# CagriCatik/RRT-MPC

Measured on NVIDIA B200. Metric: MPC QP solves/sec (horizon 50, batched), higher is better.
Workload: dtype f64

## Files before the change

rrt_mpc_b200/csrc/mpc_core.h:

```cpp
#pragma once
#include <math.h>
#include <stdint.h>

#ifdef __CUDACC__
#define MPC_HD __host__ __device__ __forceinline__
#else
#define MPC_HD inline
#endif

namespace mpc {

struct Params {
  double L, dt;
  double pq[4][4], pr[2][2], pqn[4][4];
  double u_lo[2], u_hi[2];
  double v_lo, v_hi;
  double du_lo[2], du_hi[2];
  double w_v, w_u, w_du;
  int N;
};

struct Settings {
  double eps_abs, eps_rel;
  double rho0, alpha, sigma;
// ... 1106 lines not shown
    w.act()[N + 1] = ib;
  }
  return changed;
}

MPC_HD int activity_probe_stage(const View& w, const Params& p, int k) {
  const int N = w.N;
  const double* rc = w.rec(k);
  const int old = w.act()[k];
  int bits = 0;
  const int ng = ngroups(N, k);
  const double tol = 1e-6;
  for (int g = 0; g < ng; ++g) {
    double lo, hi; group_bounds(p, w.hdr(), k, g, lo, hi);
    const double m0 = rc[R_V + 3 * g] - hi, m1 = lo - rc[R_V + 3 * g + 1], m2 = -rc[R_V + 3 * g + 2];
    const int b0 = fabs(m0) <= tol ? (old >> (3 * g)) & 1 : (m0 > 0.0);
    const int b1 = fabs(m1) <= tol ? (old >> (3 * g + 1)) & 1 : (m1 > 0.0);
    const int b2 = fabs(m2) <= tol ? (old >> (3 * g + 2)) & 1 : (m2 > 0.0);
    bits |= (b0 << (3 * g)) | (b1 << (3 * g + 1)) | (b2 << (3 * g + 2));
  }
  if (k < N) bits |= 0xF << 15;
  int changed = (old != bits);
  w.act()[k] = bits;
  if (k == 0) {
    changed |= (w.act()[N + 1] != 0xF);
    w.act()[N + 1] = 0xF;
  }
  return changed;
}

struct PolishRP {
  View w; const Params* p; double inv_delta; int zero_sol;
  MPC_HD double dyn(int k, int r) const {
    if (!act_dyn_bit(w, k, r)) return 0.0;
    const double* rc = w.rec(k);
    double b = r == 0 ? rc[R_LIN + 5] : (r == 1 ? rc[R_LIN + 6] : 0.0);
    double z[4]; StateXV xs{w}; dyn_rows(w, *p, k, xs, z);
    return (b - z[r]) * inv_delta - rc[R_YE + r];
  }
  MPC_HD double init(int r) const {
    if (!act_init_bit(w, r)) return 0.0;
    const double* h = w.hdr();
    return (h[H_X0 + r] - w.rec(0)[R_XU + r]) * inv_delta - h[H_YI + r];
  }
  MPC_HD double row(int k, int g, int r) const {
    if (!((act_group_bits(w, k, g) >> r) & 1)) return 0.0;
    double lo, hi; group_bounds(*p, w.hdr(), k, g, lo, hi);
    StateXV xs{w};
    const double* rc = w.rec(k);
    double gv = group_g(k, g, xs), sv = rc[R_S + g];
    double ax = r == 0 ? gv - sv : (r == 1 ? gv + sv : sv);
    double b = r == 0 ? hi : (r == 1 ? lo : 0.0);
    return (b - ax) * inv_delta - rc[R_V + 3 * g + r];
  }
  MPC_HD void group_vals(int k, int g, const Mode& m, double& rr_s, double& gval) const {
    double v1 = row(k, g, 0), v2 = row(k, g, 1), v3 = row(k, g, 2);
    double ps = group_ps(*p, g);
    GroupCoef c = group_coef(m, ps, act_group_bits(w, k, g));
    rr_s = -ps * w.rec(k)[R_S + g] + (-v1 + v2 + v3);
    gval = v1 + v2 - c.csg * c.mss_inv * rr_s;
  }
  Mode mode;
  MPC_HD double grp(int k, int g) const { double a, b; group_vals(k, g, mode, a, b); return b; }
};

MPC_HD void polish_rhs_stage(const View& w, const Params& p, const Mode& m, int k) {
  const int N = w.N;
  double* rc = w.rec(k);
  PolishRP rp{w, &p, m.inv_delta, 0, m};
  const int ng = ngroups(N, k);
  for (int g = 0; g < ng; ++g) {
    double rr_s, gval; rp.group_vals(k, g, m, rr_s, gval);
    rc[R_ST + g] = rr_s;
  }
  double out[6];
  gather_xu(w, p, k, rp, out);
  const int nj = k < N ? 6 : 4;
  for (int j = 0; j < nj; ++j) {
    double qj = j < 4 ? rc[R_Q + j] : 0.0;
    w.bx_set(k, j, -qj - px_entry(p, k < N, j, rc + R_XU) + out[j]);
  }
  for (int j = nj; j < 6; ++j) w.bx_set(k, j, 0.0);
}
MPC_HD void polish_dual_stage(const View& w, const Params& p, const Mode& m, int k) {
  const int N = w.N;
  double* rc = w.rec(k);
  BxXV dx{w};
  StateXV xs{w};
  const int ng = ngroups(N, k);
  for (int g = 0; g < ng; ++g) {
    double lo, hi; group_bounds(p, w.hdr(), k, g, lo, hi);
    int bits = act_group_bits(w, k, g);
    GroupCoef c = group_coef(m, group_ps(p, g), bits);
    double gd = group_g(k, g, dx);
    double ds = (rc[R_ST + g] - c.csg * gd) * c.mss_inv;
    rc[R_ST + g] = ds;
    double gv = group_g(k, g, xs), sv = rc[R_S + g];
    double ax[3] = {gv - sv, gv + sv, sv};
    double ad[3] = {gd - ds, gd + ds, ds};
    double b[3] = {hi, lo, 0.0};
    for (int r = 0; r < 3; ++r)
      if ((bits >> r) & 1) rc[R_V + 3 * g + r] += m.inv_delta * (ad[r] - (b[r] - ax[r]));
  }
  if (k < N) {
    double ax[4], ad[4]; dyn_rows(w, p, k, xs, ax); dyn_rows(w, p, k, dx, ad);
    double b[4] = {rc[R_LIN + 5], rc[R_LIN + 6], 0.0, 0.0};
    for (int r = 0; r < 4; ++r)
      if (act_dyn_bit(w, k, r)) rc[R_YE + r] += m.inv_delta * (ad[r] - (b[r] - ax[r]));
  }
  if (k == 0) {
    double* h = w.hdr();
    for (int r = 0; r < 4; ++r)
      if (act_init_bit(w, r)) h[H_YI + r] += m.inv_delta * (dx(0, r) - (h[H_X0 + r] - xs(0, r)));
  }
}
MPC_HD void polish_primal_stage(const View& w, int k) {
  double* rc = w.rec(k);
  const int nj = k < w.N ? 6 : 4;
  for (int j = 0; j < nj; ++j) rc[R_XU + j] += w.bx_get(k, j);
  const int ng = ngroups(w.N, k);
  for (int g = 0; g < ng; ++g) rc[R_S + g] += rc[R_ST + g];
}
MPC_HD void polish_zero_stage(const View& w, int k) {
  double* rc = w.rec(k);
  for (int j = 0; j < 11; ++j) rc[R_XU + j] = 0.0;
  for (int j = 0; j < 15; ++j) rc[R_V + j] = 0.0;
  for (int r = 0; r < 4; ++r) rc[R_YE + r] = 0.0;
  if (k == 0) for (int r = 0; r < 4; ++r) w.hdr()[H_YI + r] = 0.0;
}

struct PolConst {
  double invd;
  double lo[5], hi[5], ps[5];
  double mssinv[5][4];
  double up0, up1;
};
MPC_HD PolConst pol_const(const View& w, const Params& p, const Settings& s) {
  PolConst c;
  c.invd = 1.0 / s.delta;
  c.lo[0] = p.v_lo; c.hi[0] = p.v_hi;
  c.lo[1] = p.u_lo[0]; c.hi[1] = p.u_hi[0]; c.lo[2] = p.u_lo[1]; c.hi[2] = p.u_hi[1];
  c.lo[3] = p.du_lo[0]; c.hi[3] = p.du_hi[0]; c.lo[4] = p.du_lo[1]; c.hi[4] = p.du_hi[1];
  for (int g = 0; g < 5; ++g) {
    c.ps[g] = group_ps(p, g);
    for (int na = 0; na < 4; ++na) c.mssinv[g][na] = s.delta / ((c.ps[g] + s.delta) * s.delta + na);
  }
  c.up0 = w.hdr()[H_UPREV]; c.up1 = w.hdr()[H_UPREV + 1];
  return c;
}
MPC_HD double mss_pick(const PolConst& c, int g, int bits) {
  const int na = (bits & 1) + ((bits >> 1) & 1) + ((bits >> 2) & 1);
  return na == 0 ? c.mssinv[g][0] : (na == 1 ? c.mssinv[g][1] : (na == 2 ? c.mssinv[g][2] : c.mssinv[g][3]));
}
MPC_HD double pol_group_val(const PolConst& c, int g, int bits, double gv, double sv, double lo, double hi,
                            double y0, double y1, double y2, double& rr_s) {
  const double v0 = (bits & 1) ? fma(hi - (gv - sv), c.invd, -y0) : 0.0;
  const double v1 = (bits & 2) ? fma(lo - (gv + sv), c.invd, -y1) : 0.0;
  const double v2 = (bits & 4) ? fma(-sv, c.invd, -y2) : 0.0;
  rr_s = fma(-c.ps[g], sv, (v1 - v0) + v2);
  const double csg = (double)(((bits >> 1) & 1) - (bits & 1)) * c.invd;
  return (v0 + v1) - csg * mss_pick(c, g, bits) * rr_s;
}
MPC_HD void dyn_rows6(const double* lin, double dt, const double* x, const double* xn, double* z) {
  z[0] = xn[0] - (x[0] + lin[0] * x[2] + lin[1] * x[3]);
  z[1] = xn[1] - (x[1] + lin[2] * x[2] + lin[3] * x[3]);
  z[2] = xn[2] - (x[2] + lin[4] * x[5]);
  z[3] = xn[3] - (x[3] + dt * x[4]);
}

MPC_HD void polish_rhs_fast(const View& w, const Params& p, const PolConst& c, int k) {
  const int N = w.N;
  double* rc = w.rec(k);
  const bool reg = k < N;
  const int act = w.act()[k];
  double x[6];
#pragma unroll
  for (int j = 0; j < 6; ++j) x[j] = rc[R_XU + j];
  double out[6] = {0.0, 0.0, 0.0, 0.0, 0.0, 0.0};
  double ua = 0.0, ud = 0.0;
  if (k >= 1) {
    const double* rp = w.rec(k - 1);
    double xp[6], z[4];
#pragma unroll
    for (int j = 0; j < 6; ++j) xp[j] = rp[R_XU + j];
    ua = xp[4]; ud = xp[5];
    dyn_rows6(rp + R_LIN, p.dt, xp, x, z);
    const int ap = w.act()[k - 1];
    const double b[4] = {rp[R_LIN + 5], rp[R_LIN + 6], 0.0, 0.0};
#pragma unroll
    for (int r = 0; r < 4; ++r) out[r] = ((ap >> (15 + r)) & 1) ? fma(b[r] - z[r], c.invd, -rp[R_YE + r]) : 0.0;
  } else {
    const double* h = w.hdr();
    const int ai = w.act()[N + 1];
#pragma unroll
    for (int r = 0; r < 4; ++r) out[r] = ((ai >> r) & 1) ? fma(h[H_X0 + r] - x[r], c.invd, -h[H_YI + r]) : 0.0;
  }
  const double off0 = k == 0 ? c.up0 : 0.0, off1 = k == 0 ? c.up1 : 0.0;
  const double gv[5] = {x[3], x[4], x[5], x[4] - (reg ? ua : 0.0), x[5] - (reg ? ud : 0.0)};
  const double offs[5] = {0.0, 0.0, 0.0, off0, off1};
  double G[5] = {0.0, 0.0, 0.0, 0.0, 0.0};
#pragma unroll
  for (int g = 0; g < 5; ++g) {
    if (g == 0 || reg) {
      double rr_s;
      G[g] = pol_group_val(c, g, (act >> (3 * g)) & 7, gv[g], rc[R_S + g], c.lo[g] + offs[g], c.hi[g] + offs[g],
                           rc[R_V + 3 * g], rc[R_V + 3 * g + 1], rc[R_V + 3 * g + 2], rr_s);
      rc[R_ST + g] = rr_s;
    }
  }
  out[3] += G[0];
  if (reg) {
    const double* rn = w.rec(k + 1);
    double xn[6], z[4];
#pragma unroll
    for (int j = 0; j < 6; ++j) xn[j] = rn[R_XU + j];
    const double* lin = rc + R_LIN;
    dyn_rows6(lin, p.dt, x, xn, z);
    const double b[4] = {lin[5], lin[6], 0.0, 0.0};
    double d[4];
#pragma unroll
    for (int r = 0; r < 4; ++r) d[r] = ((act >> (15 + r)) & 1) ? fma(b[r] - z[r], c.invd, -rc[R_YE + r]) : 0.0;
    out[0] -= d[0];
    out[1] -= d[1];
    out[2] -= lin[0] * d[0] + lin[2] * d[1] + d[2];
    out[3] -= lin[1] * d[0] + lin[3] * d[1] + d[3];
    out[4] = G[1] + G[3] - p.dt * d[3];
    out[5] = G[2] + G[4] - lin[4] * d[2];
    if (k + 1 < N) {
      const int an = w.act()[k + 1];
#pragma unroll
      for (int i = 0; i < 2; ++i) {
        double rr_s;
        out[4 + i] -= pol_group_val(c, 3 + i, (an >> (3 * (3 + i))) & 7, xn[4 + i] - x[4 + i], rn[R_S + 3 + i], c.lo[3 + i], c.hi[3 + i],
                                    rn[R_V + 3 * (3 + i)], rn[R_V + 3 * (3 + i) + 1], rn[R_V + 3 * (3 + i) + 2], rr_s);
      }
    }
  }
  int rev; double* bp = bx_ptr(w, k, rev);
#pragma unroll
  for (int j = 0; j < 6; ++j) {
    double val = 0.0;
    if (j < 4 || reg) val = -(j < 4 ? rc[R_Q + j] : 0.0) - px_entry(p, reg, j, x) + out[j];
    bp[rev ? 5 - j : j] = val;
  }
  if (k == mid_stage(N)) {
    double* bb = w.bottom().bx(N - k);
#pragma unroll
    for (int j = 0; j < 6; ++j) bb[j] = 0.0;
  }
}

MPC_HD void polish_dual_fast(const View& w, const Params& p, const PolConst& c, int k) {
  const int N = w.N;
  double* rc = w.rec(k);
  const bool reg = k < N;
  const int act = w.act()[k];
  double x[6], dx[6];
#pragma unroll
  for (int j = 0; j < 6; ++j) x[j] = rc[R_XU + j];
  bx_load6(w, k, dx);
  double ua = 0.0, ud = 0.0, dua_ = 0.0, dud_ = 0.0;
  if (k >= 1 && reg) {
    const double* rp = w.rec(k - 1);
    ua = rp[R_XU + 4]; ud = rp[R_XU + 5];
    double dp[6]; bx_load6(w, k - 1, dp); dua_ = dp[4]; dud_ = dp[5];
  }
  const double off0 = k == 0 ? c.up0 : 0.0, off1 = k == 0 ? c.up1 : 0.0;
  const double offs[5] = {0.0, 0.0, 0.0, off0, off1};
  const double gv[5] = {x[3], x[4], x[5], x[4] - ua, x[5] - ud};
  const double gd[5] = {dx[3], dx[4], dx[5], dx[4] - dua_, dx[5] - dud_};
#pragma unroll
  for (int g = 0; g < 5; ++g) {
    if (g == 0 || reg) {
      const int bits = (act >> (3 * g)) & 7;
      const double csg = (double)(((bits >> 1) & 1) - (bits & 1)) * c.invd;
      const double ds = (rc[R_ST + g] - csg * gd[g]) * mss_pick(c, g, bits);
      rc[R_ST + g] = ds;
      const double sv = rc[R_S + g];
      if (bits & 1) rc[R_V + 3 * g] += c.invd * ((gd[g] - ds) - ((c.hi[g] + offs[g]) - (gv[g] - sv)));
      if (bits & 2) rc[R_V + 3 * g + 1] += c.invd * ((gd[g] + ds) - ((c.lo[g] + offs[g]) - (gv[g] + sv)));
      if (bits & 4) rc[R_V + 3 * g + 2] += c.invd * (ds - (0.0 - sv));
    }
  }
  if (reg) {
    const double* rn = w.rec(k + 1);
    double xn[6], dn[6], ax[4], ad[4];
#pragma unroll
    for (int j = 0; j < 6; ++j) xn[j] = rn[R_XU + j];
    bx_load6(w, k + 1, dn);
    const double* lin = rc + R_LIN;
    dyn_rows6(lin, p.dt, x, xn, ax);
    dyn_rows6(lin, p.dt, dx, dn, ad);
    const double b[4] = {lin[5], lin[6], 0.0, 0.0};
#pragma unroll
    for (int r = 0; r < 4; ++r)
      if ((act >> (15 + r)) & 1) rc[R_YE + r] += c.invd * (ad[r] - (b[r] - ax[r]));
  }
  if (k == 0) {
    double* h = w.hdr();
    const int ai = w.act()[N + 1];
#pragma unroll
    for (int r = 0; r < 4; ++r)
      if ((ai >> r) & 1) h[H_YI + r] += c.invd * (dx[r] - (h[H_X0 + r] - x[r]));
  }
}

MPC_HD void residual_fast(const View& w, const Params& p, const IterConst& c, int ymode, int k, double* r) {
  const int N = w.N;
  const double* rc = w.rec(k);
  const bool reg = k < N;
  double x[6];
#pragma unroll
  for (int j = 0; j < 6; ++j) x[j] = rc[R_XU + j];
  double aty[6] = {0.0, 0.0, 0.0, 0.0, 0.0, 0.0};
  double ua = 0.0, ud = 0.0;
  if (k >= 1) {
    const double* rp = w.rec(k - 1);
    ua = rp[R_XU + 4]; ud = rp[R_XU + 5];
#pragma unroll
    for (int q = 0; q < 4; ++q) aty[q] = rp[R_YE + q];
  } else {
    const double* h = w.hdr();
#pragma unroll
    for (int q = 0; q < 4; ++q) {
      aty[q] = h[H_YI + q];
      const double ax = x[q], b = h[H_X0 + q];
      r[0] = dmax(r[0], fabs(ax - b)); r[1] = dmax(r[1], fabs(ax)); r[2] = dmax(r[2], fabs(b));
    }
  }
  const double off0 = k == 0 ? c.up0 : 0.0, off1 = k == 0 ? c.up1 : 0.0;
  const double offs[5] = {0.0, 0.0, 0.0, off0, off1};
  const double gv[5] = {x[3], x[4], x[5], x[4] - (reg ? ua : 0.0), x[5] - (reg ? ud : 0.0)};
  double Gy[5] = {0.0, 0.0, 0.0, 0.0, 0.0};
#pragma unroll
  for (int g = 0; g < 5; ++g) {
    if (g == 0 || reg) {
      const double hi = c.hi[g] + offs[g], lo = c.lo[g] + offs[g];
      const double sv = rc[R_S + g];
      const double v0 = rc[R_V + 3 * g], v1 = rc[R_V + 3 * g + 1], v2 = rc[R_V + 3 * g + 2];
      const double ax0 = gv[g] - sv, ax1 = gv[g] + sv, ax2 = sv;
      double z0, z1, z2, y0, y1, y2;
      if (ymode) { z0 = dmin2(ax0, hi); z1 = dmax2(ax1, lo); z2 = dmax2(ax2, 0.0); y0 = v0; y1 = v1; y2 = v2; }
      else {
        z0 = dmin2(v0, hi); z1 = dmax2(v1, lo); z2 = dmax2(v2, 0.0);
        y0 = c.rho * (v0 - z0); y1 = c.rho * (v1 - z1); y2 = c.rho * (v2 - z2);
      }
      r[0] = dmax(r[0], dmax(fabs(ax0 - z0), dmax(fabs(ax1 - z1), fabs(ax2 - z2))));
      r[1] = dmax(r[1], dmax(fabs(ax0), dmax(fabs(ax1), fabs(ax2))));
      r[2] = dmax(r[2], dmax(fabs(z0), dmax(fabs(z1), fabs(z2))));
      Gy[g] = y0 + y1;
      const double px = c.ps_[g] * sv, ay = (y1 - y0) + y2;
      r[3] = dmax(r[3], fabs(px + ay)); r[4] = dmax(r[4], fabs(px)); r[5] = dmax(r[5], fabs(ay));
    }
  }
  aty[3] += Gy[0];
  if (reg) {
    const double* rn = w.rec(k + 1);
    const double* lin = rc + R_LIN;
    double xn[4], ax[4];
#pragma unroll
    for (int j = 0; j < 4; ++j) xn[j] = rn[R_XU + j];
    ax[0] = xn[0] - (x[0] + lin[0] * x[2] + lin[1] * x[3]);
    ax[1] = xn[1] - (x[1] + lin[2] * x[2] + lin[3] * x[3]);
    ax[2] = xn[2] - (x[2] + lin[4] * x[5]);
    ax[3] = xn[3] - (x[3] + p.dt * x[4]);
    const double b[4] = {lin[5], lin[6], 0.0, 0.0};
#pragma unroll
    for (int q = 0; q < 4; ++q) {
      r[0] = dmax(r[0], fabs(ax[q] - b[q])); r[1] = dmax(r[1], fabs(ax[q])); r[2] = dmax(r[2], fabs(b[q]));
    }
    const double d0 = rc[R_YE + 0], d1 = rc[R_YE + 1], d2 = rc[R_YE + 2], d3 = rc[R_YE + 3];
    aty[0] -= d0;
    aty[1] -= d1;
    aty[2] -= lin[0] * d0 + lin[2] * d1 + d2;
    aty[3] -= lin[1] * d0 + lin[3] * d1 + d3;
    aty[4] = Gy[1] + Gy[3] - p.dt * d3;
    aty[5] = Gy[2] + Gy[4] - lin[4] * d2;
    if (k + 1 < N) {
#pragma unroll
      for (int i = 0; i < 2; ++i) {
        const double v0 = rn[R_V + 3 * (3 + i)], v1 = rn[R_V + 3 * (3 + i) + 1];
        double y0, y1;
        if (ymode) { y0 = v0; y1 = v1; }
        else { y0 = c.rho * (v0 - dmin2(v0, c.hi[3 + i])); y1 = c.rho * (v1 - dmax2(v1, c.lo[3 + i])); }
        aty[4 + i] -= y0 + y1;
      }
    }
  }
#pragma unroll
  for (int j = 0; j < 6; ++j) {
    if (j < 4 || reg) {
      const double px = px_entry(p, reg, j, x), qj = j < 4 ? rc[R_Q + j] : 0.0;
      r[3] = dmax(r[3], fabs(px + qj + aty[j])); r[4] = dmax(r[4], fabs(px)); r[5] = dmax(r[5], fabs(aty[j]));
      r[6] = dmax(r[6], fabs(qj));
    }
  }
}

MPC_HD void save_stage(const View& w, int k, double* g) {
  const double* rc = w.rec(k);
  double* o = g + 30 * k;
  for (int j = 0; j < 30; ++j) o[j] = rc[R_XU + j];
}
MPC_HD void load_stage(const View& w, int k, const double* g) {
  double* rc = w.rec(k);
  const double* o = g + 30 * k;
  for (int j = 0; j < 30; ++j) rc[R_XU + j] = o[j];
}

}
```

rrt_mpc_b200/csrc/mpc_drv.h:

```cpp
#pragma once
#include "mpc_solve.h"

namespace mpc {

struct Drv {
  double rho, pri, dua, se_abs, se_rel;
  Residuals res;
  int status, it, retries, n_rho, n_fac, n_solve, n_pol, nb;
  int finished, need_restore, need_factor, need_rhs;
  int phase;
  int last, check, adapt, converged;
  int pass, acc;
  double pp, dd;
  IterConst ic;
};
enum { PH_ADMM = 0, PH_POLISH = 1 };

template <class Exec>
MPC_HD void drv_begin(Exec& ex, const View& w, const Params& p, const Settings& s, const ProblemIO& io, Drv& d) {
  const int N = w.N, NS = N + 1;
  ex.tag(0);
  ex.single([&]() {
    double* h = w.hdr();
    for (int i = 0; i < 4; ++i) h[H_X0 + i] = io.x0[i];
    for (int i = 0; i < 2; ++i) h[H_UPREV + i] = io.u_prev ? io.u_prev[i] : 0.0;
    for (int i = 0; i < N + 2; ++i) w.act()[i] = 0;
    unwrap_window(io.ref, NS, w.scratch());
  });
  ex.stages(NS, [&](int k) { setup_stage(w, p, k, io.ref, w.scratch()); });
  d.rho = s.rho0;
  const double rho_slot = (s.warm_start && io.warm) ? io.warm[30 * NS + 4] : 0.0;
  if (rho_slot >= s.rho_min && rho_slot <= s.rho_max) {
    ex.stages(NS, [&](int k) { load_stage(w, k, io.warm); });
    ex.single([&]() { for (int r = 0; r < 4; ++r) w.hdr()[H_YI + r] = io.warm[30 * NS + r]; });
    d.rho = rho_slot;
  } else {
    ex.stages(NS, [&](int k) { cold_start_stage(w, p, k); });
  }
  d.ic = iter_const(w, p, s, d.rho);
  d.status = STATUS_UNSOLVED; d.it = 0;
  d.res.pri = d.res.dua = 1e300; d.res.eps_p = d.res.eps_d = 0.0; d.res.sp = d.res.sd = 0.0; d.res.nz = d.res.nq = 0.0;
  d.pri = d.dua = 1e300;
  d.se_abs = s.eps_abs; d.se_rel = s.eps_rel;
  d.retries = s.polish_retry;
  d.n_rho = d.n_fac = d.n_solve = d.n_pol = 0; d.nb = 0;
  d.finished = 0; d.need_restore = 0; d.need_factor = 1; d.need_rhs = 1;
  d.phase = PH_ADMM;
  d.last = d.check = d.adapt = d.converged = 0; d.pass = d.acc = 0; d.pp = d.dd = 0.0;
}

template <class Exec>
MPC_HD void drv_prepare(Exec& ex, const View& w, const Params& p, const Settings& s, Drv& d) {
  const int NS = w.N + 1;
  const OEView oe = oe_view(w);
  if (d.need_factor) {
    const Mode mode = admm_mode(d.rho, s);
    ex.tag(5); ex.oe_factor(w, p, mode, oe); ++d.n_fac;
    d.ic = iter_const(w, p, s, d.rho);
    d.need_factor = 0;
    d.need_rhs = 1;
  }
  if (d.need_rhs) {
    ex.tag(6);
    const IterConst ic = d.ic;
#pragma unroll 1
    for (int par = 1; par >= 0; --par) ex.stages_par(NS, par, [&](int k) { admm_rhs_stage_oe(w, p, ic, oe, k); });
    d.need_rhs = 0;
  }
  int nb = s.max_iter - d.it;
  if (s.check_termination > 0) { const int n = s.check_termination - d.it % s.check_termination; if (n < nb) nb = n; }
  if (s.adaptive_rho && s.adaptive_rho_interval > 0) { const int n = s.adaptive_rho_interval - d.it % s.adaptive_rho_interval; if (n < nb) nb = n; }
  d.nb = nb < 1 ? 1 : nb;
  ex.tag(2);
}

template <class Exec>
MPC_HD void drv_after(Exec& ex, const View& w, const Params& p, const Settings& s, const ProblemIO& io, Drv& d) {
  const int NS = w.N + 1;
  const bool can_polish = s.polish_passes > 0 && io.warm && io.scratch;
  const bool polishing = d.phase == PH_POLISH;
  if (!polishing) {
    d.it += d.nb; d.n_solve += d.nb;
    d.last = d.it >= s.max_iter;
    d.check = d.last || ((s.check_termination > 0) && (d.it % s.check_termination == 0));
    d.adapt = !d.last && s.adaptive_rho && (s.adaptive_rho_interval > 0) && (d.it % s.adaptive_rho_interval == 0);
    if (!(d.check || d.adapt)) return;
  }
  Settings se = s; se.eps_abs = d.se_abs; se.eps_rel = d.se_rel;
  const IterConst ic = d.ic;
  ex.tag(polishing ? 12 : 3);
  const Residuals rr = compute_residuals(ex, w, p, se, ic, polishing ? 1 : 0);
  bool run_pass = false, polish_end = false, settled = false;
  int rejected = 0;
  if (!polishing) {
    d.res = rr;
    d.pri = rr.pri; d.dua = rr.dua;
    if (d.check) {
      const bool last = d.last;
      const bool converged = rr.pri <= rr.eps_p && rr.dua <= rr.eps_d;
      if (converged && d.status == STATUS_UNSOLVED) d.status = STATUS_SOLVED;
      if (last && d.status == STATUS_UNSOLVED) {
        const double ep10 = 10.0 * s.eps_abs + 10.0 * s.eps_rel * rr.nz, ed10 = 10.0 * s.eps_abs + 10.0 * s.eps_rel * rr.nq;
        d.status = (rr.pri <= ep10 && rr.dua <= ed10) ? STATUS_SOLVED_INACCURATE : STATUS_MAX_ITER;
      }
      bool attempt = converged || (last && d.status == STATUS_SOLVED);
      if (!attempt && !last && s.early_polish && can_polish) {
        ex.tag(15);
        const int changed = ex.any(NS, [&](int k) { return activity_probe_stage(w, p, k); });
        attempt = (!changed || s.early_polish >= 2) && d.it >= s.early_polish_start;
      }
      if (attempt || last) {
        ex.tag(8);
        if (io.warm) {
          ex.stages(NS, [&](int k) { save_stage(w, k, io.warm); });
          const double rho = d.rho;
          ex.single([&]() {
            for (int r = 0; r < 4; ++r) io.warm[30 * NS + r] = w.hdr()[H_YI + r];
            io.warm[30 * NS + 4] = (rr.pri < 1e300 && rr.dua < 1e300) ? rho : 0.0;
          });
        }
        if (attempt && can_polish) {
          if (io.fsave && !last && !(converged && d.retries <= 0)) ex.stages(oe_doubles(w.N), [&](int i) { oe_save_word(w, i, io.fsave); });
          d.converged = converged;
          d.pass = 0; d.acc = 0;
          d.pp = rr.pri; d.dd = rr.dua;
          run_pass = true;
        } else {
          d.finished = 1;
        }
      }
    }
  } else {
    const int pass = d.pass;
    const double pp = d.pp, dd = d.dd, nz = d.res.nz, nq = d.res.nq;
    bool ok;
    if (pass == 0) ok = (rr.pri < pp && rr.dua < dd) || (rr.pri < pp && dd < 1e-10) || (rr.dua < dd && pp < 1e-10);
    else ok = rr.pri <= dmax(10.0 * pp, 1e-9 * dmax(1.0, nz)) && rr.dua <= dmax(10.0 * dd, 1e-9 * dmax(1.0, nq));
    if (ok) {
      d.pp = rr.pri; d.dd = rr.dua; d.acc = pass + 1;
      d.pass = pass + 1;
      if (d.pass < s.polish_passes) run_pass = true; else polish_end = true;
    } else {
      rejected = pass == 0 ? 1 : 2;
      polish_end = true;
    }
  }
  if (run_pass) {
    const int pass = d.pass;
    ex.tag(9);
    if (pass > 0) {
      ex.stages(NS, [&](int k) { save_stage(w, k, io.scratch); });
      ex.single([&]() { for (int r = 0; r < 4; ++r) io.scratch[30 * NS + r] = w.hdr()[H_YI + r]; });
    }
    const double rho = d.rho;
    const int changed = ex.any(NS, [&](int k) { return polish_activity_stage(w, p, rho, pass == 0, k); });
    if (pass > 0 && !changed) {
      settled = true;
      polish_end = true;
    } else {
      const Mode pm = polish_mode(s);
      const PolConst pc = pol_const(w, p, s);
      ex.stages(NS, [&](int k) { polish_zero_stage(w, k); });
      ex.stages(NS, [&](int k) { assemble_stage(w, p, pm, k); });
      ex.tag(10); ex.factor(w); ++d.n_fac;
      ex.tag(11);
      for (int step = 0; step <= s.polish_refine_iter; ++step) {
        ex.stages(NS, [&](int k) { polish_rhs_fast(w, p, pc, k); });
        ex.solve(w); ++d.n_solve;
        ex.stages(NS, [&](int k) { polish_dual_fast(w, p, pc, k); });
        ex.stages(NS, [&](int k) { polish_primal_stage(w, k); });
      }
      ex.tag(12);
      d.phase = PH_POLISH;
      return;
    }
  }
  if (polish_end) {
    d.phase = PH_ADMM;
    if (rejected == 2) {
      ex.stages(NS, [&](int k) { load_stage(w, k, io.scratch); });
      ex.single([&]() { for (int r = 0; r < 4; ++r) w.hdr()[H_YI + r] = io.scratch[30 * NS + r]; });
    }
    const int acc = d.acc;
    const double pp = d.pp, dd = d.dd;
    if (acc > 0) { d.pri = pp; d.dua = dd; }
    d.n_pol = acc;
    const bool clean = acc > 0 && (settled || s.polish_passes == 1) && pp <= 1e-9 * dmax(1.0, d.res.nz) && dd <= 1e-9 * dmax(1.0, d.res.nq);
    const bool converged = d.converged;
    if (clean) { d.status = STATUS_SOLVED; d.finished = 1; }
    else if (d.last || (converged && d.retries <= 0)) {
      d.finished = 1;
      if (d.n_pol == 0) d.need_restore = 1;
    } else {
      if (converged) { --d.retries; d.se_abs *= 0.1; d.se_rel *= 0.1; }
      d.n_pol = 0;
      ex.tag(13);
      ex.stages(NS, [&](int k) { load_stage(w, k, io.warm); });
      ex.single([&]() { for (int r = 0; r < 4; ++r) w.hdr()[H_YI + r] = io.warm[30 * NS + r]; });
      if (io.fsave) { ex.stages(oe_doubles(w.N), [&](int i) { oe_restore_word(w, i, io.fsave); }); d.need_rhs = 1; }
      else d.need_factor = 1;
    }
  }
  if (d.adapt && !d.finished) {
    const Residuals res = d.res;
    double rho_new = d.rho * sqrt(res.sp / (res.sd + 1e-10));
    rho_new = fmin(fmax(rho_new, s.rho_min), s.rho_max);
    if (rho_new > d.rho * s.adaptive_rho_tolerance || rho_new < d.rho / s.adaptive_rho_tolerance) {
      const double rho_old = d.rho;
      ex.stages(NS, [&](int k) { rescale_v_stage(w, p, rho_old, rho_new, k); });
      d.rho = rho_new; ++d.n_rho;
      d.need_factor = 1;
    }
  }
}

template <class Exec>
MPC_HD void drv_finish(Exec& ex, const View& w, const ProblemIO& io, const Drv& d) {
  const int N = w.N, NS = N + 1;
  ex.tag(7);
  if (d.need_restore) {
    ex.stages(NS, [&](int k) { load_stage(w, k, io.warm); });
    ex.single([&]() { for (int r = 0; r < 4; ++r) w.hdr()[H_YI + r] = io.warm[30 * NS + r]; });
  }
  ex.stages(NS, [&](int k) {
    const double* rc = w.rec(k);
    for (int j = 0; j < 4; ++j) io.Xp[j * NS + k] = rc[R_XU + j];
    if (k < N) { io.Up[k] = rc[R_XU + 4]; io.Up[N + k] = rc[R_XU + 5]; }
    if (k == 0) {
      io.u0[0] = rc[R_XU + 4]; io.u0[1] = rc[R_XU + 5];
      *io.status = d.status; *io.iters = d.it;
      if (io.pri_res) *io.pri_res = d.pri;
      if (io.dua_res) *io.dua_res = d.dua;
      if (io.info) { io.info[0] = d.n_rho; io.info[1] = d.n_fac; io.info[2] = d.n_pol; io.info[3] = d.n_solve; }
    }
  });
}

template <class Exec>
MPC_HD void solve_problem_reg(Exec& ex, const View& w, const Params& p, const Settings& s, const ProblemIO& io) {
  Drv d;
  drv_begin(ex, w, p, s, io, d);
  const OEView oe = oe_view(w);
  while (!d.finished) {
    if (d.phase == PH_ADMM) {
      drv_prepare(ex, w, p, s, d);
      ex.admm_block(w, p, d.ic, oe, d.nb);
    }
    drv_after(ex, w, p, s, io, d);
  }
  drv_finish(ex, w, io, d);
}

}
```

rrt_mpc_b200/csrc/mpc_exec.cuh:

```cuda
#pragma once
#include <cuda_runtime.h>
#include "mpc_solve.h"

namespace mpc {

template <int PIPE>
__device__ __forceinline__ void chain_twisted_lanes(bool active, bool bottom, int partner, const View& w) {
  double a[6] = {0.0, 0.0, 0.0, 0.0, 0.0, 0.0}, o[6], xm[6] = {0.0, 0.0, 0.0, 0.0, 0.0, 0.0};
  const HalfView h = bottom ? w.bottom() : w.top();
  if (active) half_forward<PIPE>(h, a);
  __syncwarp();
#pragma unroll
  for (int j = 0; j < 6; ++j) o[j] = __shfl_sync(0xffffffffu, a[5 - j], partner);
  if (active && !bottom) {
#pragma unroll
    for (int j = 0; j < 6; ++j) a[j] += o[j];
    middle_solve(w, a, xm);
  }
  __syncwarp();
#pragma unroll
  for (int j = 0; j < 6; ++j) o[j] = __shfl_sync(0xffffffffu, xm[5 - j], partner);
  if (active) half_backward<PIPE>(h, bottom ? o : xm);
  __syncwarp();
}
// ... 221 lines not shown
      MPC_BTAG(22);
    }
    MPC_BAR();
    if (!ev && on) reg_expand(w, p, c, oe, k, R, T);
    MPC_BAR();
    MPC_BTAG(23);
    if (ev && on) reg_gather_even(w, k, T);
    if (on) reg_update<STATE>(w, p, c, k, R, T);
    MPC_BAR();
    MPC_BTAG(24);
    if (on) reg_rhs<STATE>(w, p, c, oe, k, R, T);
    MPC_BAR();
    MPC_BTAG(25);
    if (ev && on) reg_fixup(w, p, c, k, T);
    if (sweeper) __syncwarp();
  }
#ifdef MPC_TIMING
  if (sweeper && lane == 0 && tags) for (int q = 0; q < 7; ++q) atomicAdd(&tags[20 + q], (unsigned long long)tacc[q]);
#endif
  MPC_BAR();
  if (on) reg_store<STATE>(w, k, R);
  MPC_BAR();
}

template <int WPP>
struct GroupExec {
  int lane, warp;
  GroupShared* sh;
  __device__ __forceinline__ int grp() const { return warp / WPP; }
  __device__ __forceinline__ int sub() const { return warp % WPP; }
  __device__ __forceinline__ int gl() const { return sub() * 32 + lane; }
  __device__ __forceinline__ bool chain_warp() const { return WPP == 1 || sub() == ((grp() >> 1) & 1); }
  __device__ __forceinline__ void group_sync() const {
    if (WPP == 1) __syncwarp();
    else asm volatile("bar.sync %0, %1;" ::"r"(1 + grp()), "r"(32 * WPP) : "memory");
  }
#ifdef MPC_TIMING
  long long t_last = 0; int t_cur = 0; unsigned long long* tags = nullptr;
  __device__ __forceinline__ void tag(int n) {
    const long long now = clock64();
    if (gl() == 0 && t_last && tags) atomicAdd(&tags[t_cur], (unsigned long long)(now - t_last));
    t_last = now; t_cur = n;
  }
#else
  __device__ __forceinline__ void tag(int) {}
#endif
  template <class Fn> __device__ __forceinline__ void stages(int n, Fn f) {
    for (int k = gl(); k < n; k += 32 * WPP) f(k);
    group_sync();
  }
  template <class Fn> __device__ __forceinline__ void stages_par(int n, int par, Fn f) {
    for (int k = 2 * gl() + par; k < n; k += 64 * WPP) f(k);
    group_sync();
  }
  template <class Fn> __device__ __forceinline__ void single(Fn f) {
    if (gl() == 0) f();
    group_sync();
  }
  template <class Fn> __device__ __forceinline__ void reduce_max(int n, double* r, int nr, Fn f) {
    for (int i = 0; i < nr; ++i) r[i] = 0.0;
    for (int k = gl(); k < n; k += 32 * WPP) f(k, r);
    for (int i = 0; i < nr; ++i) {
      double v = r[i];
#pragma unroll
      for (int o = 16; o > 0; o >>= 1) v = fmax(v, __shfl_xor_sync(0xffffffffu, v, o));
      r[i] = v;
    }
    if (WPP > 1) {
      if (lane == 0) for (int i = 0; i < nr; ++i) sh->red[sub()][i] = r[i];
      group_sync();
      for (int i = 0; i < nr; ++i) r[i] = fmax(sh->red[0][i], sh->red[1][i]);
    }
    group_sync();
  }
  template <class Fn> __device__ __forceinline__ int any(int n, Fn f) {
    int a = 0;
    for (int k = gl(); k < n; k += 32 * WPP) a |= f(k);
    a = __any_sync(0xffffffffu, a);
    if (WPP > 1) {
      if (lane == 0) sh->anyv[sub()] = a;
      group_sync();
      a = sh->anyv[0] | sh->anyv[1];
    }
    group_sync();
    return a;
  }
  __device__ __forceinline__ int fetch(int* counter) {
    if (WPP == 1) return next_problem_warp(counter, lane);
    if (gl() == 0) sh->next = atomicAdd(counter, 1);
    group_sync();
    const int b = sh->next;
    group_sync();
    return b;
  }
  __device__ __forceinline__ void solve(const View& w) {
    if (chain_warp()) chain_twisted_lanes<0>(lane < 2, lane == 1, lane ^ 1, w);
    group_sync();
  }
  __device__ __forceinline__ void oe_factor(const View& w, const Params& p, const Mode& m, const OEView& oe) {
    stages_par(w.N + 1, 1, [&](int k) { oe_factor_odd(w, p, m, oe, k); });
    stages_par(w.N + 1, 0, [&](int k) { oe_factor_even(w, p, m, oe, k); });
    if (chain_warp()) oe_factor_lanes(lane, w, oe);
    group_sync();
  }
  __device__ __forceinline__ void oe_forward(const View& w, const OEView& oe) {
    if (chain_warp()) oe_forward_lanes(lane, w, oe);
    group_sync();
  }
  __device__ __forceinline__ void oe_backward(const View& w, const OEView& oe) {
    if (chain_warp()) oe_backward_lanes(lane, w, oe);
    group_sync();
  }
  __device__ __forceinline__ void pair_pass(const View& w, const Params& p, const IterConst& c, const OEView& oe) {
    const unsigned full = 0xffffffffu;
    const bool on = lane < pair_lanes(w.N);
    PairCtx cx;
#pragma unroll
    for (int j = 0; j < 6; ++j) { cx.xe[j] = 0.0; cx.xo[j] = 0.0; cx.xn[j] = 0.0; cx.be[j] = 0.0; cx.bo[j] = 0.0; cx.t[j] = 0.0; }
#pragma unroll
    for (int j = 0; j < 4; ++j) { cx.de[j] = 0.0; cx.dd[j] = 0.0; }
#pragma unroll
    for (int j = 0; j < 5; ++j) { cx.Ge[j] = 0.0; cx.Go[j] = 0.0; }
    if (on) pair_expand(w, p, c, oe, lane, cx);
    double ua = __shfl_up_sync(full, cx.xo[4], 1), ud = __shfl_up_sync(full, cx.xo[5], 1);
    if (lane == 0) { ua = 0.0; ud = 0.0; }
    if (on) pair_update(w, p, c, lane, cx, ua, ud);
    double dprev[4], rnext[2], tprev[6];
#pragma unroll
    for (int r = 0; r < 4; ++r) dprev[r] = __shfl_up_sync(full, cx.dd[r], 1);
#pragma unroll
    for (int i = 0; i < 2; ++i) rnext[i] = __shfl_down_sync(full, cx.Ge[3 + i], 1);
    if (on) pair_rhs(w, p, c, oe, lane, cx, dprev, rnext);
#pragma unroll
    for (int j = 0; j < 6; ++j) tprev[j] = __shfl_up_sync(full, cx.t[j], 1);
    if (on) pair_fixup(w, p, c, lane, cx, tprev);
    group_sync();
  }
  __device__ __forceinline__ void admm_block(const View& w, const Params& p, const IterConst& c, const OEView&, int nb) {
    if (gl() == 0) sh->drv.ic = c;
    group_sync();
#ifdef MPC_TIMING
    unsigned long long* tg = tags;
#else
    unsigned long long* tg = nullptr;
#endif
    reg_block_run<0, WPP>(w.base, w.N, w.fpad, w.xpad, p.dt, &sh->drv.ic, nb, lane, chain_warp() ? 1 : 0, 1 + grp(), tg);
  }
  __device__ __forceinline__ void factor(const View& w) {
    if (chain_warp()) factor_twisted_lanes(lane, w, 0, max(half_top(w.N), half_bot(w.N)), true);
    group_sync();
  }
};

}
```

Baseline: 459,700.

## Add GPU-specialised polish refinement loop with precomputed per-stage pointers

Adds a per-stage PolStage descriptor that precomputes record pointers, RHS row pointers with stride, activity bits and the selected mss values, and new polish rhs/dual/primal routines that take it. On the GPU GroupExec path, a polish_refine overload maps each stage to one lane, computes the descriptor once per refine step and runs the three stage passes with explicit group syncs instead of separate generic ex.stages launches. The intent is to cut repeated index and pointer work and per-pass scheduling overhead in the polishing phase. It adds register pressure for the cached descriptor, and it assumes the group has at least N+1 lanes.

```diff
diff --git a/rrt_mpc_b200/csrc/mpc_core.h b/rrt_mpc_b200/csrc/mpc_core.h
--- a/rrt_mpc_b200/csrc/mpc_core.h
+++ b/rrt_mpc_b200/csrc/mpc_core.h
@@ -1282,14 +1282,14 @@
   const int na = (bits & 1) + ((bits >> 1) & 1) + ((bits >> 2) & 1);
   return na == 0 ? c.mssinv[g][0] : (na == 1 ? c.mssinv[g][1] : (na == 2 ? c.mssinv[g][2] : c.mssinv[g][3]));
 }
-MPC_HD double pol_group_val(const PolConst& c, int g, int bits, double gv, double sv, double lo, double hi,
+MPC_HD double pol_group_val(const PolConst& c, int g, int bits, double mss, double gv, double sv, double lo, double hi,
                             double y0, double y1, double y2, double& rr_s) {
   const double v0 = (bits & 1) ? fma(hi - (gv - sv), c.invd, -y0) : 0.0;
   const double v1 = (bits & 2) ? fma(lo - (gv + sv), c.invd, -y1) : 0.0;
   const double v2 = (bits & 4) ? fma(-sv, c.invd, -y2) : 0.0;
   rr_s = fma(-c.ps[g], sv, (v1 - v0) + v2);
   const double csg = (double)(((bits >> 1) & 1) - (bits & 1)) * c.invd;
-  return (v0 + v1) - csg * mss_pick(c, g, bits) * rr_s;
+  return (v0 + v1) - csg * mss * rr_s;
 }
 MPC_HD void dyn_rows6(const double* lin, double dt, const double* x, const double* xn, double* z) {
   z[0] = xn[0] - (x[0] + lin[0] * x[2] + lin[1] * x[3]);
@@ -1333,7 +1333,7 @@
   for (int g = 0; g < 5; ++g) {
     if (g == 0 || reg) {
       double rr_s;
-      G[g] = pol_group_val(c, g, (act >> (3 * g)) & 7, gv[g], rc[R_S + g], c.lo[g] + offs[g], c.hi[g] + offs[g],
+      G[g] = pol_group_val(c, g, (act >> (3 * g)) & 7, mss_pick(c, g, (act >> (3 * g)) & 7), gv[g], rc[R_S + g], c.lo[g] + offs[g], c.hi[g] + offs[g],
                            rc[R_V + 3 * g], rc[R_V + 3 * g + 1], rc[R_V + 3 * g + 2], rr_s);
       rc[R_ST + g] = rr_s;
     }
@@ -1361,7 +1361,7 @@
 #pragma unroll
       for (int i = 0; i < 2; ++i) {
         double rr_s;
-        out[4 + i] -= pol_group_val(c, 3 + i, (an >> (3 * (3 + i))) & 7, xn[4 + i] - x[4 + i], rn[R_S + 3 + i], c.lo[3 + i], c.hi[3 + i],
+        out[4 + i] -= pol_group_val(c, 3 + i, (an >> (3 * (3 + i))) & 7, mss_pick(c, 3 + i, (an >> (3 * (3 + i))) & 7), xn[4 + i] - x[4 + i], rn[R_S + 3 + i], c.lo[3 + i], c.hi[3 + i],
                                     rn[R_V + 3 * (3 + i)], rn[R_V + 3 * (3 + i) + 1], rn[R_V + 3 * (3 + i) + 2], rr_s);
       }
     }
@@ -1432,6 +1432,196 @@
 #pragma unroll
     for (int r = 0; r < 4; ++r)
       if ((ai >> r) & 1) h[H_YI + r] += c.invd * (dx[r] - (h[H_X0 + r] - x[r]));
+  }
+}
+
+struct PolStage {
+  double* rc; const double* rp; const double* rn;
+  double* bx; const double* bxp; const double* bxn;
+  int bst, bstp, bstn;
+  double* bmid;
+  int k, act, ap, an, ai;
+  double mss[5], mssn[2];
+};
+MPC_HD void pol_row(const View& w, int k, double*& r, int& st) {
+  const bool rev = k > mid_stage(w.N);
+  r = rev ? w.bottom().bx(w.N - k) + 5 : w.top().bx(k);
+  st = rev ? -1 : 1;
+}
+MPC_HD PolStage pol_stage(const View& w, const PolConst& c, int k) {
+  const int N = w.N;
+  const int kp = k >= 1 ? k - 1 : k, kn = k < N ? k + 1 : k;
+  PolStage s;
+  s.k = k;
+  s.rc = w.rec(k); s.rp = w.rec(kp); s.rn = w.rec(kn);
+  double* r;
+  pol_row(w, k, s.bx, s.bst);
+  pol_row(w, kp, r, s.bstp); s.bxp = r;
+  pol_row(w, kn, r, s.bstn); s.bxn = r;
+  s.bmid = k == mid_stage(N) ? w.bottom().bx(N - k) : nullptr;
+  const int* a = w.act();
+  s.act = a[k]; s.ap = a[kp]; s.an = k + 1 < N ? a[k + 1] : 0; s.ai = a[N + 1];
+#pragma unroll
+  for (int g = 0; g < 5; ++g) s.mss[g] = mss_pick(c, g, (s.act >> (3 * g)) & 7);
+#pragma unroll
+  for (int i = 0; i < 2; ++i) s.mssn[i] = mss_pick(c, 3 + i, (s.an >> (3 * (3 + i))) & 7);
+  return s;
+}
+
+MPC_HD void polish_rhs_fast(const View& w, const Params& p, const PolConst& c, const PolStage& st) {
+  const int N = w.N, k = st.k;
+  double* rc = st.rc;
+  const bool reg = k < N;
+  const int act = st.act;
+  double x[6];
+#pragma unroll
+  for (int j = 0; j < 6; ++j) x[j] = rc[R_XU + j];
+  double out[6] = {0.0, 0.0, 0.0, 0.0, 0.0, 0.0};
+  double ua = 0.0, ud = 0.0;
+  if (k >= 1) {
+    const double* rp = st.rp;
+    double xp[6], z[4];
+#pragma unroll
+    for (int j = 0; j < 6; ++j) xp[j] = rp[R_XU + j];
+    ua = xp[4]; ud = xp[5];
+    dyn_rows6(rp + R_LIN, p.dt, xp, x, z);
+    const int ap = st.ap;
+    const double b[4] = {rp[R_LIN + 5], rp[R_LIN + 6], 0.0, 0.0};
+#pragma unroll
+    for (int r = 0; r < 4; ++r) out[r] = ((ap >> (15 + r)) & 1) ? fma(b[r] - z[r], c.invd, -rp[R_YE + r]) : 0.0;
+  } else {
+    const double* h = w.hdr();
+    const int ai = st.ai;
+#pragma unroll
+    for (int r = 0; r < 4; ++r) out[r] = ((ai >> r) & 1) ? fma(h[H_X0 + r] - x[r], c.invd, -h[H_YI + r]) : 0.0;
+  }
+  const double off0 = k == 0 ? c.up0 : 0.0, off1 = k == 0 ? c.up1 : 0.0;
+  const double gv[5] = {x[3], x[4], x[5], x[4] - (reg ? ua : 0.0), x[5] - (reg ? ud : 0.0)};
+  const double offs[5] = {0.0, 0.0, 0.0, off0, off1};
+  double G[5] = {0.0, 0.0, 0.0, 0.0, 0.0};
+#pragma unroll
+  for (int g = 0; g < 5; ++g) {
+    if (g == 0 || reg) {
+      double rr_s;
+      G[g] = pol_group_val(c, g, (act >> (3 * g)) & 7, st.mss[g], gv[g], rc[R_S + g], c.lo[g] + offs[g], c.hi[g] + offs[g],
+                           rc[R_V + 3 * g], rc[R_V + 3 * g + 1], rc[R_V + 3 * g + 2], rr_s);
+      rc[R_ST + g] = rr_s;
+    }
+  }
+  out[3] += G[0];
+  if (reg) {
+    const double* rn = st.rn;
+    double xn[6], z[4];
+#pragma unroll
+    for (int j = 0; j < 6; ++j) xn[j] = rn[R_XU + j];
+    const double* lin = rc + R_LIN;
+    dyn_rows6(lin, p.dt, x, xn, z);
+    const double b[4] = {lin[5], lin[6], 0.0, 0.0};
+    double d[4];
+#pragma unroll
+    for (int r = 0; r < 4; ++r) d[r] = ((act >> (15 + r)) & 1) ? fma(b[r] - z[r], c.invd, -rc[R_YE + r]) : 0.0;
+    out[0] -= d[0];
+    out[1] -= d[1];
+    out[2] -= lin[0] * d[0] + lin[2] * d[1] + d[2];
+    out[3] -= lin[1] * d[0] + lin[3] * d[1] + d[3];
+    out[4] = G[1] + G[3] - p.dt * d[3];
+    out[5] = G[2] + G[4] - lin[4] * d[2];
+    if (k + 1 < N) {
+      const int an = st.an;
+#pragma unroll
+      for (int i = 0; i < 2; ++i) {
+        double rr_s;
+        out[4 + i] -= pol_group_val(c, 3 + i, (an >> (3 * (3 + i))) & 7, st.mssn[i], xn[4 + i] - x[4 + i], rn[R_S + 3 + i], c.lo[3 + i], c.hi[3 + i],
+                                    rn[R_V + 3 * (3 + i)], rn[R_V + 3 * (3 + i) + 1], rn[R_V + 3 * (3 + i) + 2], rr_s);
+      }
+    }
+  }
+  double* bp = st.bx;
+  const int bs = st.bst;
+#pragma unroll
+  for (int j = 0; j < 6; ++j) {
+    double val = 0.0;
+    if (j < 4 || reg) val = -(j < 4 ? rc[R_Q + j] : 0.0) - px_entry(p, reg, j, x) + out[j];
+    bp[j * bs] = val;
+  }
+  if (st.bmid) {
+#pragma unroll
+    for (int j = 0; j < 6; ++j) st.bmid[j] = 0.0;
+  }
+}
+
+MPC_HD void polish_dual_fast(const View& w, const Params& p, const PolConst& c, const PolStage& st) {
+  const int N = w.N, k = st.k;
+  double* rc = st.rc;
+  const bool reg = k < N;
+  const int act = st.act;
+  double x[6], dx[6];
+#pragma unroll
+  for (int j = 0; j < 6; ++j) x[j] = rc[R_XU + j];
+#pragma unroll
+  for (int j = 0; j < 6; ++j) dx[j] = st.bx[j * st.bst];
+  double ua = 0.0, ud = 0.0, dua_ = 0.0, dud_ = 0.0;
+  if (k >= 1 && reg) {
+    const double* rp = st.rp;
+    ua = rp[R_XU + 4]; ud = rp[R_XU + 5];
+    dua_ = st.bxp[4 * st.bstp]; dud_ = st.bxp[5 * st.bstp];
+  }
+  const double off0 = k == 0 ? c.up0 : 0.0, off1 = k == 0 ? c.up1 : 0.0;
+  const double offs[5] = {0.0, 0.0, 0.0, off0, off1};
+  const double gv[5] = {x[3], x[4], x[5], x[4] - ua, x[5] - ud};
+  const double gd[5] = {dx[3], dx[4], dx[5], dx[4] - dua_, dx[5] - dud_};
+#pragma unroll
+  for (int g = 0; g < 5; ++g) {
+    if (g == 0 || reg) {
+      const int bits = (act >> (3 * g)) & 7;
+      const double csg = (double)(((bits >> 1) & 1) - (bits & 1)) * c.invd;
+      const double ds = (rc[R_ST + g] - csg * gd[g]) * st.mss[g];
+      rc[R_ST + g] = ds;
+      const double sv = rc[R_S + g];
+      if (bits & 1) rc[R_V + 3 * g] += c.invd * ((gd[g] - ds) - ((c.hi[g] + offs[g]) - (gv[g] - sv)));
+      if (bits & 2) rc[R_V + 3 * g + 1] += c.invd * ((gd[g] + ds) - ((c.lo[g] + offs[g]) - (gv[g] + sv)));
+      if (bits & 4) rc[R_V + 3 * g + 2] += c.invd * (ds - (0.0 - sv));
+    }
+  }
+  if (reg) {
+    const double* rn = st.rn;
+    double xn[6], dn[6], ax[4], ad[4];
+#pragma unroll
+    for (int j = 0; j < 6; ++j) xn[j] = rn[R_XU + j];
+#pragma unroll
+    for (int j = 0; j < 6; ++j) dn[j] = st.bxn[j * st.bstn];
+    const double* lin = rc + R_LIN;
+    dyn_rows6(lin, p.dt, x, xn, ax);
+    dyn_rows6(lin, p.dt, dx, dn, ad);
+    const double b[4] = {lin[5], lin[6], 0.0, 0.0};
+#pragma unroll
+    for (int r = 0; r < 4; ++r)
+      if ((act >> (15 + r)) & 1) rc[R_YE + r] += c.invd * (ad[r] - (b[r] - ax[r]));
+  }
+  if (k == 0) {
+    double* h = w.hdr();
+    const int ai = st.ai;
+#pragma unroll
+    for (int r = 0; r < 4; ++r)
+      if ((ai >> r) & 1) h[H_YI + r] += c.invd * (dx[r] - (h[H_X0 + r] - x[r]));
+  }
+}
+MPC_HD void polish_primal_fast(const View& w, const PolStage& st) {
+  double* rc = st.rc;
+  const int nj = st.k < w.N ? 6 : 4;
+  for (int j = 0; j < nj; ++j) rc[R_XU + j] += st.bx[j * st.bst];
+  const int ng = ngroups(w.N, st.k);
+  for (int g = 0; g < ng; ++g) rc[R_S + g] += rc[R_ST + g];
+}
+
+template <class Exec>
+MPC_HD void polish_refine(Exec& ex, const View& w, const Params& p, const PolConst& c, int steps) {
+  const int NS = w.N + 1;
+  for (int step = 0; step < steps; ++step) {
+    ex.stages(NS, [&](int k) { polish_rhs_fast(w, p, c, pol_stage(w, c, k)); });
+    ex.tag(19); ex.solve(w); ex.tag(11);
+    ex.stages(NS, [&](int k) { polish_dual_fast(w, p, c, pol_stage(w, c, k)); });
+    ex.stages(NS, [&](int k) { polish_primal_fast(w, pol_stage(w, c, k)); });
   }
 }
 
diff --git a/rrt_mpc_b200/csrc/mpc_drv.h b/rrt_mpc_b200/csrc/mpc_drv.h
--- a/rrt_mpc_b200/csrc/mpc_drv.h
+++ b/rrt_mpc_b200/csrc/mpc_drv.h
@@ -164,12 +164,8 @@
       ex.stages(NS, [&](int k) { assemble_stage(w, p, pm, k); });
       ex.tag(10); ex.factor(w); ++d.n_fac;
       ex.tag(11);
-      for (int step = 0; step <= s.polish_refine_iter; ++step) {
-        ex.stages(NS, [&](int k) { polish_rhs_fast(w, p, pc, k); });
-        ex.solve(w); ++d.n_solve;
-        ex.stages(NS, [&](int k) { polish_dual_fast(w, p, pc, k); });
-        ex.stages(NS, [&](int k) { polish_primal_stage(w, k); });
-      }
+      const int steps = s.polish_refine_iter >= 0 ? s.polish_refine_iter + 1 : 0;
+      polish_refine(ex, w, p, pc, steps); d.n_solve += steps;
       ex.tag(12);
       d.phase = PH_POLISH;
       return;
diff --git a/rrt_mpc_b200/csrc/mpc_exec.cuh b/rrt_mpc_b200/csrc/mpc_exec.cuh
--- a/rrt_mpc_b200/csrc/mpc_exec.cuh
+++ b/rrt_mpc_b200/csrc/mpc_exec.cuh
@@ -397,4 +397,21 @@
   }
 };
 
-}
+template <int WPP>
+__device__ __forceinline__ void polish_refine(GroupExec<WPP>& ex, const View& w, const Params& p, const PolConst& c, int steps) {
+  const int k = ex.gl();
+  const bool on = k <= w.N;
+#pragma unroll 1
+  for (int step = 0; step < steps; ++step) {
+    const PolStage st = pol_stage(w, c, on ? k : w.N);
+    if (on) polish_rhs_fast(w, p, c, st);
+    ex.group_sync();
+    ex.tag(19); ex.solve(w); ex.tag(11);
+    if (on) polish_dual_fast(w, p, c, st);
+    ex.group_sync();
+    if (on) polish_primal_fast(w, st);
+    ex.group_sync();
+  }
+}
+
+}
```

Result: no change. 461,400, median of 6 (+0.4%).
